# genometools/vstree

Measured on AMD Instinct MI355X. Metric: queries/sec (100 bp queries, vmatch -mum -l 20 semantics, 3 Gbp ESA index resident in HBM), higher is better.
Workload: dtype u8; 1 GPU; 3 Gbp synthetic DNA index, 10 M x 100 bp queries per GPU, -mum -l 20; index_bp=3000000000, queries_per_gpu=10000000, query_len=100, minlen=20, prefixlength=13, index_bytes_hbm=115012207262, reads_in_hbm=two bits per symbol, 32 bytes per read (vsa_pack_reads), parallelism=index replicated, queries sharded x1

## Files before the change

### vstree_amd/csrc/candidate_sort.inc

```

#define VSA_CS_CAP 4096
#define VSA_CS_ITEMS (VSA_CS_CAP / VSA_BLOCK)
#define VSA_CS_BINBITS 11
#define VSA_CS_BINS (1u << VSA_CS_BINBITS)
#define VSA_CS_BINLIMIT 256
#define VSA_CS_OVERFLOW 2u

struct CsGeometry
{
  unsigned int shift, lenbits;
  uint64_t nbuckets;
};

struct CsRegions
{
  const void *vals;
  const uint64_t *keys;
  const unsigned long long *cursors;
  uint64_t cap;
  uint64_t total;
};

struct CsFirst
{
  const uint32_t *fmlen;
  const uint64_t *fmdb;
  uint64_t nq, seqoffset;
  uint32_t packbits, valbits;
};

struct CsSources
{
  CsRegions reg[2];
  CsFirst first;
};

template <typename VAL, bool SMALL>
struct CsForm
{
  using Entry = typename std::conditional<SMALL, uint64_t, ulonglong2>::type;

  static __device__ __forceinline__ Entry make(uint64_t key, VAL val,
                                               const CsGeometry &g)
  {
    if constexpr (SMALL)
    {
      const uint64_t low = key & ((1ull << (g.shift + g.lenbits)) - 1);
      return (low << 32) | (uint64_t) val;
    } else
    {
      return make_ulonglong2(key, (uint64_t) val);
    }
  }
  static __device__ __forceinline__ uint64_t sub(const Entry &e,
                                                 const CsGeometry &g)
  {
    if constexpr (SMALL)
    {
      return e >> (32 + g.lenbits);
    } else
    {
      return (e.x >> g.lenbits) & ((1ull << g.shift) - 1);
    }
  }
  static __device__ __forceinline__ uint64_t key(const Entry &e,
                                                 uint64_t bucket,
                                                 const CsGeometry &g)
  {
    if constexpr (SMALL)
    {
      return (bucket << (g.shift + g.lenbits)) | (e >> 32);
    } else
    {
      return e.x;
    }
  }
  static __device__ __forceinline__ VAL val(const Entry &e)
  {
    if constexpr (SMALL)
    {
      return (VAL) e;
    } else
    {
      return (VAL) e.y;
    }
  }
};

struct CsTiles
{
  uint32_t group[2], ngroups[2];
};

#define VSA_CS_SCATTER_BLOCK 1024
#define VSA_CS_TILE_ITEMS 8
#define VSA_CS_TILE (VSA_CS_SCATTER_BLOCK * VSA_CS_TILE_ITEMS)
#define VSA_CS_MAXBUCKETS 12288

template <typename VAL, typename Fn>
__device__ __forceinline__ void
vsa_cs_foreach(const CsRegions &r, uint64_t wg, uint32_t group, Fn fn)
{
  const VAL *vals = static_cast<const VAL *>(r.vals);
  const uint32_t wave = threadIdx.x >> 6, lane = threadIdx.x & 63u;
  const uint64_t shard = wg * group + wave;
  if (wave >= group || shard >= VSA_CURSOR_SHARDS)
  {
    return;
  }
  uint64_t count = r.cursors[shard * VSA_CURSOR_STRIDE];
  count = count < r.cap ? count : r.cap;
  const uint64_t at = shard * r.cap;
  for (uint64_t i = lane; i < count; i += 64)
  {
    fn(r.keys[at + i], vals[at + i]);
  }
}

template <typename VAL, bool SMALL>
__global__ void __launch_bounds__(VSA_CS_SCATTER_BLOCK)
k_cs_scatter(CsSources src, CsTiles t, CsGeometry g,
             uint32_t *__restrict__ counts,
             typename CsForm<VAL, SMALL>::Entry *__restrict__ staging)
{
  extern __shared__ uint32_t cs_hist[];
  const uint32_t nb = (uint32_t) g.nbuckets;
  auto bucket = [&](uint64_t key) {
    const uint64_t b = (key >> g.lenbits) >> g.shift;
    return (uint32_t) (b < nb ? b : nb - 1);
  };
  const uint32_t lane = threadIdx.x & 63u;
  auto count = [&](uint64_t key, VAL) {
    const uint32_t b = bucket(key);
    const uint64_t active = __ballot(1);
    const uint32_t b0 = (uint32_t) __builtin_amdgcn_readfirstlane((int) b);
    if (__ballot(b == b0) == active)
    {
      if ((int) lane == __ffsll((unsigned long long) active) - 1)
      {
        atomicAdd(&cs_hist[b0], (uint32_t) __popcll(active));
      }
    } else
    {
      atomicAdd(&cs_hist[b], 1u);
    }
  };
  auto place = [&](uint64_t key, VAL val) {
    const uint32_t b = bucket(key);
    const uint64_t active = __ballot(1);
    const uint32_t b0 = (uint32_t) __builtin_amdgcn_readfirstlane((int) b);
    uint32_t rank;
    if (__ballot(b == b0) == active)
    {
      uint32_t base = 0;
      if ((int) lane == __ffsll((unsigned long long) active) - 1)
      {
        base = atomicAdd(&cs_hist[b0], (uint32_t) __popcll(active));
      }
      rank = (uint32_t) __builtin_amdgcn_readfirstlane((int) base) +
             (uint32_t) __popcll(active & ((1ull << lane) - 1));
    } else
    {
      rank = atomicAdd(&cs_hist[b], 1u);
    }
    if (rank < VSA_CS_CAP)
    {
      staging[(uint64_t) b * VSA_CS_CAP + rank] =
          CsForm<VAL, SMALL>::make(key, val, g);
    }
  };
  uint64_t wg = vsa_bid();
  int set = 0;
  while (set < 2 && wg >= t.ngroups[set])
  {
    wg -= t.ngroups[set++];
  }
  const CsFirst &f = src.first;
  uint64_t key[VSA_CS_TILE_ITEMS];
  uint32_t have = 0;
  const uint64_t q0 = wg * VSA_CS_TILE + threadIdx.x;
  if (set == 2)
  {
    uint32_t len[VSA_CS_TILE_ITEMS];
#pragma unroll
    for (int u = 0; u < VSA_CS_TILE_ITEMS; u++)
    {
      const uint64_t q = q0 + (uint64_t) u * VSA_CS_SCATTER_BLOCK;
      len[u] = q < f.nq ? f.fmlen[q] : 0;
      key[u] = q < f.nq ? f.fmdb[q] : 0;
    }
#pragma unroll
    for (int u = 0; u < VSA_CS_TILE_ITEMS; u++)
    {
      key[u] = (key[u] << f.packbits) | (((1ull << f.packbits) - 1) - len[u]);
      have |= len[u] != 0 ? 1u << u : 0u;
    }
  }
  for (uint32_t b = threadIdx.x; b < nb; b += VSA_CS_SCATTER_BLOCK)
  {
    cs_hist[b] = 0;
  }
  __syncthreads();
  if (set == 2)
  {
#pragma unroll
    for (int u = 0; u < VSA_CS_TILE_ITEMS; u++)
    {
      if ((have >> u) & 1u)
      {
        count(key[u], 0);
      }
    }
  } else
  {
    vsa_cs_foreach<VAL>(set == 0 ? src.reg[0] : src.reg[1], wg, t.group[set],
                        count);
  }
  __syncthreads();
  for (uint32_t b = threadIdx.x; b < nb; b += VSA_CS_SCATTER_BLOCK)
  {
    const uint32_t c = cs_hist[b];
    if (c != 0)
    {
      cs_hist[b] = atomicAdd(&counts[b], c);
    }
  }
  __syncthreads();
  if (set == 2)
  {
#pragma unroll
    for (int u = 0; u < VSA_CS_TILE_ITEMS; u++)
    {
      if ((have >> u) & 1u)
      {
        const uint64_t q = q0 + (uint64_t) u * VSA_CS_SCATTER_BLOCK;
        place(key[u], sizeof(VAL) == 4 ? (VAL) (q << f.valbits)
                                       : (VAL) ((q + f.seqoffset) << 16));
      }
    }
  } else
  {
    vsa_cs_foreach<VAL>(set == 0 ? src.reg[0] : src.reg[1], wg, t.group[set],
                        place);
  }
}

__global__ void __launch_bounds__(VSA_BLOCK)
k_cs_scan(const uint32_t *__restrict__ counts, uint64_t nbuckets,
          uint64_t *__restrict__ starts, unsigned int *__restrict__ flag)
{
  __shared__ uint64_t sh[VSA_BLOCK / 64 + 1];
  uint64_t run = 0;
  uint32_t largest = 0;
  for (uint64_t b = 0; b < nbuckets; b += VSA_BLOCK * VSA_FT_SCANITEMS)
  {
    const uint64_t i0 = b + (uint64_t) threadIdx.x * VSA_FT_SCANITEMS;
    uint32_t v[VSA_FT_SCANITEMS];
    uint64_t mine = 0;
#pragma unroll
    for (int k = 0; k < VSA_FT_SCANITEMS; k++)
    {
      v[k] = i0 + k < nbuckets ? counts[i0 + k] : 0;
      mine += v[k];
      largest = v[k] > largest ? v[k] : largest;
    }
    uint64_t total;
    uint64_t ex = run + vsa_block_exscan<0>(mine, sh, total);
#pragma unroll
    for (int k = 0; k < VSA_FT_SCANITEMS; k++)
    {
      if (i0 + k < nbuckets)
      {
        starts[i0 + k] = ex;
      }
      ex += v[k];
    }
    run += total;
  }
  if (largest > VSA_CS_CAP)
  {
    atomicOr(flag, VSA_CS_OVERFLOW);
  }
}

template <typename VAL, bool SMALL>
__global__ void __launch_bounds__(VSA_BLOCK)
k_cs_sort(const typename CsForm<VAL, SMALL>::Entry *__restrict__ staging,
          const uint32_t *__restrict__ counts,
          const uint64_t *__restrict__ starts,
          unsigned int *__restrict__ flag, CsGeometry g, uint64_t ncand,
          uint64_t *__restrict__ k2, VAL *__restrict__ v2)
{
  using F = CsForm<VAL, SMALL>;
  using Entry = typename F::Entry;
  __shared__ Entry buf[VSA_CS_CAP];
  __shared__ uint32_t bins[VSA_CS_BINS];
  uint64_t *sh = reinterpret_cast<uint64_t *>(buf);
  uint32_t *toobig = reinterpret_cast<uint32_t *>(buf) + 32;
  const uint64_t b = vsa_bid();
  if (b >= g.nbuckets)
  {
    return;
  }
  const uint32_t c = counts[b];
  const uint64_t start = starts[b];
  if (c == 0 || c > VSA_CS_CAP || start + c > ncand)
  {
    return;
  }
  if (threadIdx.x == 0)
  {
    *toobig = (*flag & VSA_CS_OVERFLOW) != 0 ? 1u : 0u;
  }
  const unsigned int binshift =
      g.shift > VSA_CS_BINBITS ? g.shift - VSA_CS_BINBITS : 0;
  for (uint32_t k = threadIdx.x; k < VSA_CS_BINS; k += VSA_BLOCK)
  {
    bins[k] = 0;
  }
  __syncthreads();
  if (*toobig != 0)
  {
    return;
  }
  Entry e[VSA_CS_ITEMS];
#pragma unroll
  for (int k = 0; k < VSA_CS_ITEMS; k++)
  {
    const uint32_t i = k * VSA_BLOCK + threadIdx.x;
    if (i < c)
    {
      e[k] = staging[b * VSA_CS_CAP + i];
      atomicAdd(&bins[F::sub(e[k], g) >> binshift], 1u);
    }
  }
  __syncthreads();
  {
    constexpr int PER = VSA_CS_BINS / VSA_BLOCK;
    uint32_t v[PER];
    uint64_t mine = 0;
#pragma unroll
    for (int j = 0; j < PER; j++)
    {
      v[j] = bins[threadIdx.x * PER + j];
      mine += v[j];
    }
    uint64_t total;
    uint32_t ex = (uint32_t) vsa_block_exscan<0>(mine, sh, total);
#pragma unroll
    for (int j = 0; j < PER; j++)
    {
      bins[threadIdx.x * PER + j] = ex;
      ex += v[j];
    }
  }
  __syncthreads();
  {
    constexpr int PER = VSA_CS_BINS / VSA_BLOCK;
    uint32_t big = 0;
#pragma unroll
    for (int j = 0; j < PER; j++)
    {
      const uint32_t x = threadIdx.x * PER + j;
      const uint32_t end = x + 1 < VSA_CS_BINS ? bins[x + 1] : c;
      big |= end - bins[x] > VSA_CS_BINLIMIT ? 1u : 0u;
    }
    if (big != 0)
    {
      *toobig = 1;
    }
    __syncthreads();
    if (*toobig != 0)
    {
      if (threadIdx.x == 0)
      {
        atomicOr(flag, VSA_CS_OVERFLOW);
      }
      return;
    }
    __syncthreads();
  }
#pragma unroll
  for (int k = 0; k < VSA_CS_ITEMS; k++)
  {
    const uint32_t i = k * VSA_BLOCK + threadIdx.x;
    if (i < c)
    {
      buf[atomicAdd(&bins[F::sub(e[k], g) >> binshift], 1u)] = e[k];
    }
  }
  __syncthreads();
  for (uint32_t p = threadIdx.x; p < c; p += VSA_BLOCK)
  {
    const Entry m = buf[p];
    const uint64_t sm = F::sub(m, g);
    const uint32_t x = (uint32_t) (sm >> binshift);
    const uint32_t first = x > 0 ? bins[x - 1] : 0, end = bins[x];
    uint32_t r = first;
    for (uint32_t j = first; j < end; j++)
    {
      const uint64_t sj = F::sub(buf[j], g);
      r += (sj < sm || (sj == sm && j < p)) ? 1u : 0u;
    }
    if (r < c)
    {
      k2[start + r] = F::key(m, b, g);
      v2[start + r] = F::val(m);
    }
  }
}

inline CsGeometry cs_geometry(uint64_t textlen, uint64_t ncand,
                              unsigned int lenbits, unsigned int dbbits)
{
  CsGeometry g;
  const unsigned __int128 room =
      (unsigned __int128) (VSA_CS_CAP / 2) * ((unsigned __int128) textlen + 1);
  unsigned int s = 0;
  while (s < dbbits && s < 63 && ((unsigned __int128) ncand << (s + 1)) <= room)
  {
    s++;
  }
  g.shift = s;
  g.lenbits = lenbits;
  g.nbuckets = (textlen >> s) + 1;
  return g;
}

template <typename VAL>
int candidate_bucketsort(const CsSources &src, uint64_t ncand,
                         uint64_t textlen, unsigned int lenbits,
                         unsigned int dbbits, uint64_t *k2, VAL *v2,
                         unsigned int *flag, hipStream_t stream,
                         CsGeometry *used)
{
  const CsGeometry g = cs_geometry(textlen, ncand, lenbits, dbbits);
  if (g.nbuckets > VSA_CS_MAXBUCKETS)
  {
    return -100;
  }
  const bool small = sizeof(VAL) == 4 && g.shift + lenbits <= 32;
  DevBuf counts, starts, staging;
  if (counts.alloc(g.nbuckets * 4) || starts.alloc(g.nbuckets * 8) ||
      staging.alloc(g.nbuckets * VSA_CS_CAP * (small ? 8 : 16)))
  {
    return -100;
  }
  VSA_HIP(hipMemsetAsync(counts.p, 0, g.nbuckets * 4, stream));
  CsTiles t = CsTiles();
  uint64_t nwg = 0;
  for (int s = 0; s < 2; s++)
  {
    if (src.reg[s].keys != nullptr)
    {
      const uint64_t per = src.reg[s].total / VSA_CURSOR_SHARDS + 1;
      t.group[s] = (uint32_t) std::min<uint64_t>(
          std::max<uint64_t>(VSA_CS_TILE / per, 1), VSA_CS_SCATTER_BLOCK / 64);
      t.ngroups[s] = (VSA_CURSOR_SHARDS + t.group[s] - 1) / t.group[s];
      nwg += t.ngroups[s];
    }
  }
  if (src.first.fmlen != nullptr)
  {
    nwg += (src.first.nq + VSA_CS_TILE - 1) / VSA_CS_TILE;
  }
  const dim3 sg = vsa_grid(nwg), bg = vsa_grid(g.nbuckets);
  auto run = [&](auto sm) {
    using F = CsForm<VAL, decltype(sm)::value>;
    using Entry = typename F::Entry;
    k_cs_scatter<VAL, decltype(sm)::value>
        <<<sg, VSA_CS_SCATTER_BLOCK, g.nbuckets * 4, stream>>>(
            src, t, g, counts.as<uint32_t>(), staging.as<Entry>());
    k_cs_scan<<<1, VSA_BLOCK, 0, stream>>>(counts.as<uint32_t>(), g.nbuckets,
                                           starts.as<uint64_t>(), flag);
    k_cs_sort<VAL, decltype(sm)::value><<<bg, VSA_BLOCK, 0, stream>>>(
        staging.as<Entry>(), counts.as<uint32_t>(), starts.as<uint64_t>(),
        flag, g, ncand, k2, v2);
  };
  if constexpr (sizeof(VAL) == 4)
  {
    if (small)
    {
      run(std::true_type());
    } else
    {
      run(std::false_type());
    }
  } else
  {
    run(std::false_type());
  }
  VSA_HIP(hipGetLastError());
  *used = g;
  return 0;
}
```

### vstree_amd/csrc/esa_search.hip

```cpp
#include "search_host.hpp"
#include <rocprim/rocprim.hpp>
#include <type_traits>

#include "search_complete.inc"
#include "search_query.inc"
#include "mum_workplan.inc"
#include "mem_workplan.inc"
#include "mum_filter.inc"
#include "candidate_sort.inc"
#include <atomic>


namespace
{


enum class Form
{
  Ref,
  Deep,
  Staged,
  Rows,
  Windows
};
// ... 642 lines not shown
        ix.lcp, ix.suf, index->n, st.searchlength, index->repbits);
    VSA_HIP(hipGetLastError());
    index->repleast = st.searchlength;
  }
  const Form first = pickform(index, st.queries, st.qs, Stage::MemFirst,
                              st.searchlength);
  PlanEmit em;
  if (alloc_first(st) || first_pass(st, ix, first, nullptr) ||
      plan_emit(st, VSA_PLAN_ROUNDS, &em))
  {
    return -100;
  }
  k_mem_plan<IDX><<<gridfor(nq), VSA_BLOCK, 0, st.stream>>>(
      ix, st.qs, st.perquery, st.searchlength, st.wfirste.as<uint32_t>(),
      st.wfmdb.as<uint64_t>(), index->repbits, st.wcount.as<uint32_t>(),
      st.wplan.as<PlanRanges>(), em);
  VSA_HIP(hipGetLastError());
  VSA_HIP(plan_summary(st));
  st.fromplan = true;
  st.plansearches = nq;
  return 0;
}

int dump_planfile(QueryRun &st, const char *pf)
{
  const uint64_t k = std::min<uint64_t>(st.queries->nq, 65536);
  std::vector<uint32_t> hc(k), hp(k * VSA_PLAN_RANGES);
  VSA_HIP(hipMemcpyAsync(hc.data(), st.wcount.p, k * 4,
                         hipMemcpyDeviceToHost, st.stream));
  VSA_HIP(hipMemcpyAsync(hp.data(), st.wplan.p, k * sizeof(PlanRanges),
                         hipMemcpyDeviceToHost, st.stream));
  VSA_HIP(hipStreamSynchronize(st.stream));
  if (FILE *f = fopen(pf, "wb"))
  {
    for (uint64_t q = 0; q < k; q++)
    {
      (void) fwrite(&hc[q], 4, 1, f);
      (void) fwrite(&hp[q * VSA_PLAN_RANGES], 4, VSA_PLAN_RANGES, f);
    }
    fclose(f);
  }
  return 0;
}

template <typename IDX>
int mum_plan(QueryRun &st, const DevIndex<IDX> &ix)
{
  const uint64_t nq = st.queries->nq;
  if (alloc_first(st) || st.wlist.alloc(nq * 4))
  {
    return -100;
  }
  VSA_HIP(hipMemsetAsync(st.wcount.as<uint32_t>() + nq, 0, 4, st.stream));
  const uint64_t nb = blocksfor(nq), nbr = vsa_grid_blocks(nb);
  DevBuf bcount;
  if (bcount.alloc((nbr + 1) * 8) || st.wboffset.alloc((nbr + 1) * 8))
  {
    return -100;
  }
  VSA_HIP(hipMemsetAsync(bcount.as<uint64_t>() + nb, 0, 8, st.stream));
  if (first_pass(st, ix, st.form, bcount.as<uint64_t>()))
  {
    return -100;
  }
  VSA_HIP(rocprim_run(st.wtemp, [&](void *p, size_t &tb) {
    return rocprim::exclusive_scan(p, tb, bcount.as<uint64_t>(),
                                   st.wboffset.as<uint64_t>(), (uint64_t) 0,
                                   (size_t) (nb + 1), rocprim::plus<uint64_t>(),
                                   st.stream);
  }));
  k_wanted_fill<<<vsa_grid(nb), VSA_BLOCK, 0, st.stream>>>(
      st.wcount.as<uint32_t>(), nq, 0u, st.wboffset.as<uint64_t>(),
      st.wlist.as<uint32_t>());
  VSA_HIP(hipGetLastError());
  st.nlistword = st.wboffset.as<uint64_t>() + nb;
  PlanEmit em = PlanEmit();
  if (st.form != Form::Ref && plan_emit(st, VSA_PLAN_ROUNDS - 1, &em))
  {
    return -100;
  }
  withform(st.form, [&](auto deep, auto, auto rows, auto) {
    k_mum_plan<IDX, deep, deep, rows><<<gridfor(nq), VSA_BLOCK, 0, st.stream>>>(
        ix, st.qs, st.wlist.as<uint32_t>(), st.nlistword, st.searchlength,
        st.wfirste.as<uint32_t>(), st.wcount.as<uint32_t>(),
        st.wplan.as<PlanRanges>(), em);
  });
  if (st.planemit)
  {
    VSA_HIP(plan_summary(st));
  }
  VSA_HIP(hipGetLastError());
  const char *pf = getenv("VSA_DEBUG_PLANFILE");
  if (pf != nullptr && dump_planfile(st, pf))
  {
    return -100;
  }
  st.fromplan = true;
  return 0;
}

template <typename IDX>
void launch_search(QueryRun &st, const DevIndex<IDX> &ix,
                   uint64_t nplanblocks)
{
  withform(st.form, [&](auto deep, auto, auto rows, auto) {
    auto planned = [&](auto mum) {
      k_query_search_planned<IDX, 256, deep, rows, mum>
          <<<vsa_grid(nplanblocks), 256, 0, st.stream>>>(
              ix, st.qs, st.dbase, st.perquery, st.wplan.as<PlanRanges>(),
              st.wcount.as<uint32_t>(), st.searchlength,
              st.rawout.as<vsa_match>(), st.rawkeys.as<uint64_t>(),
              st.shardcap, VSA_CURSOR_SHARDS - 1,
              st.cursor.as<unsigned long long>(), st.rec.packbits,
              st.rec.valbits, st.blocksum.as<unsigned long long>());
    };
    auto unplanned = [&](auto mum) {
      k_query_search<IDX, mum, deep, 256>
          <<<vsa_grid((st.nitems + 255) / 256), 256, 0, st.stream>>>(
              ix, st.qs, st.dbase, st.perquery, st.nitems, st.searchlength,
              st.rawout.as<vsa_match>(), st.rawkeys.as<uint64_t>(),
              st.shardcap, VSA_CURSOR_SHARDS - 1,
              st.cursor.as<unsigned long long>(), st.rec.packbits,
              st.rec.valbits);
    };
    if (st.fromplan && st.domum)
    {
      planned(std::true_type());
    } else if (st.fromplan)
    {
      if constexpr (deep && !rows)
      {
        planned(std::false_type());
      }
    } else if (st.nitems > 0 && st.domum)
    {
      unplanned(std::true_type());
    } else if (st.nitems > 0)
    {
      unplanned(std::false_type());
    }
  });
}

template <typename IDX>
int search(QueryRun &st, const DevIndex<IDX> &ix)
{
  const uint32_t nshards = VSA_CURSOR_SHARDS;
  const uint64_t nplanblocks = (st.queries->nq + 255) / 256;
  size_t rbytes = 0;
  if (st.fromplan)
  {
    if (st.blocksum.alloc((vsa_grid_blocks(nplanblocks) + 1) * 8))
    {
      return -100;
    }
    VSA_HIP(rocprim::reduce(nullptr, rbytes,
                            st.blocksum.as<unsigned long long>(),
                            (unsigned long long *) nullptr, 0ull,
                            (size_t) nplanblocks,
                            rocprim::plus<unsigned long long>(), st.stream));
    if (st.rtemp.alloc(rbytes))
    {
      return -100;
    }
  }
  if (st.cursor.alloc((size_t) nshards * VSA_CURSOR_STRIDE * 8) ||
      st.doff.alloc(nshards * 8) || st.summary.alloc(5 * 8))
  {
    return -100;
  }
  st.shardcap =
      std::max<uint64_t>((st.queries->nq * 2 / nshards) * 5 / 4 + 64, 256);
  uint64_t maxshard = 0;
  for (int attempt = 0; attempt < 2; attempt++)
  {
    if (st.rawout.alloc(nshards * st.shardcap * st.rec.recsize) ||
        st.rawkeys.alloc(nshards * st.shardcap * 8))
    {
      return -100;
    }
    VSA_HIP(hipMemsetAsync(st.cursor.p, 0,
                           (size_t) nshards * VSA_CURSOR_STRIDE * 8,
                           st.stream));
    st.tsearch.start();
    launch_search(st, ix, nplanblocks);
    st.tsearch.stop();
    VSA_HIP(hipGetLastError());
    if (st.fromplan)
    {
      VSA_HIP(rocprim::reduce(st.rtemp.p, rbytes,
                              st.blocksum.as<unsigned long long>(),
                              st.summary.as<unsigned long long>() + 4, 0ull,
                              (size_t) nplanblocks,
                              rocprim::plus<unsigned long long>(), st.stream));
    }
    const uint64_t *sm = st.summary.as<uint64_t>();
    VSA_HIP(shard_summary(st.cursor.as<unsigned long long>(), nshards,
                          st.doff.as<uint64_t>(), st.summary.as<uint64_t>(),
                          st.stream));
    const Fetch f[7] = {{sm, 8}, {sm + 1, 8}, {sm + 2, 8}, {sm + 3, 8},
                        {sm + 4, 8}, {st.planemit ? st.psummary.p : sm, 8},
                        {st.nlistword != nullptr ? st.nlistword : sm, 8}};
    uint64_t got[7];
    if (fetchwords(st.stream, f, 7, got))
    {
      return -100;
    }
    if (st.nlistword != nullptr)
    {
      st.nfirst = got[6] >> 32;
      st.plansearches = 2 * (got[6] & 0xFFFFFFFFull);
    }
    st.nplan = st.planemit ? got[5] : 0;
    st.needed = got[0];
    maxshard = got[1];
    st.plannedwork = st.fromplan ? got[4] : 0;
    st.searchms += st.tsearch.ms();
    if (maxshard <= st.shardcap)
    {
      return 0;
    }
    st.shardcap = maxshard;
  }
  VSA_ERROR("match buffer overflow: %llu > %llu",
            (unsigned long long) maxshard, (unsigned long long) st.shardcap);
  return -5;
}

int compact(QueryRun &st)
{
  const uint64_t total = st.needed + st.nplan + st.nfirst;
  if (total == 0)
  {
    return 0;
  }
  if (st.out.alloc(total * st.rec.recsize) || st.keys.alloc(total * 8) ||
      (st.nplan > 0 &&
       compact_into(st.rec, st.prawout, st.prawkeys, st.pcap, st.pcursor,
                    st.pdoff, st.out, st.keys, st.needed, st.stream)) ||
      (st.needed > 0 &&
       compact_into(st.rec, st.rawout, st.rawkeys, st.shardcap, st.cursor,
                    st.doff, st.out, st.keys, 0, st.stream)))
  {
    return -100;
  }
  if (st.nfirst > 0)
  {
    k_append_first<<<gridfor(st.queries->nq), VSA_BLOCK, 0, st.stream>>>(
        st.wfmlen.as<uint32_t>(), st.wfmdb.as<uint64_t>(),
        st.wboffset.as<uint64_t>(), st.queries->nq, st.perquery, st.dbase,
        st.qs.seqoffset, st.needed + st.nplan, st.out.as<vsa_match>(),
        st.keys.as<uint64_t>(), st.rec.packbits, st.rec.valbits);
    VSA_HIP(hipGetLastError());
  }
  st.needed = total;
  return 0;
}

#define VSA_CS_MINPAIRS (1u << 14)

std::atomic<uint64_t> g_cs_runs{0}, g_cs_overflows{0}, g_cs_longruns{0},
    g_cs_shift{0}, g_cs_buckets{0};

bool feedsbuckets(const QueryRun &st)
{
  const uint64_t total = st.needed + st.nplan + st.nfirst;
  const uint32_t tune = st.index->tune;
  if (!(st.domum && !st.domumcand && st.rec.packed && (tune & 4u) == 0 &&
        total > 0 && (total >= VSA_CS_MINPAIRS || (tune & 8u) != 0) &&
        cs_geometry(st.index->n, total, st.rec.lenbits, st.rec.dbbits)
                .nbuckets <= VSA_CS_MAXBUCKETS))
  {
    return false;
  }
  if ((tune & 8u) == 0 && st.index->cs_skip > 0)
  {
    st.index->cs_skip--;
    return false;
  }
  return true;
}

template <typename VAL>
int mumfilter_buckets(QueryRun &st, DevBuf &mums, MumCounts *c)
{
  const RecordForm &rec = st.rec;
  const uint64_t total = st.needed + st.nplan + st.nfirst;
  CsSources src = CsSources();
  if (st.needed > 0)
  {
    src.reg[0] = {st.rawout.p, st.rawkeys.as<uint64_t>(),
                  st.cursor.as<unsigned long long>(), st.shardcap, st.needed};
  }
  if (st.nplan > 0)
  {
    src.reg[1] = {st.prawout.p, st.prawkeys.as<uint64_t>(),
                  st.pcursor.as<unsigned long long>(), st.pcap, st.nplan};
  }
  if (st.nfirst > 0)
  {
    src.first = {st.wfmlen.as<uint32_t>(), st.wfmdb.as<uint64_t>(),
                 st.queries->nq, st.qs.seqoffset, rec.packbits, rec.valbits};
  }
  SortedPairs s;
  CsGeometry g;
  if (s.alloc(total, sizeof(VAL), mums))
  {
    return -100;
  }
  VSA_HIP(hipMemsetAsync(s.flag.p, 0, 8, st.stream));
  if (candidate_bucketsort<VAL>(src, total, st.index->n, rec.lenbits,
                                rec.dbbits, s.k2.as<uint64_t>(),
                                s.v2.as<VAL>(), s.flag.as<unsigned int>(),
                                st.stream, &g))
  {
    return -100;
  }
  g_cs_runs++;
  g_cs_shift = g.shift;
  g_cs_buckets = g.nbuckets;
  const PairRecord<VAL> pr = {rec.lenbits, rec.valbits,
                              sizeof(VAL) == 4 ? st.qs.seqoffset : 0};
  return mumfilter_tiles<false>(s, rec.lenbits, 0, pr, st.stream, mums, c);
}

int finish(QueryRun &st, vsa_result *res, uint64_t *mumsum)
{
  const RecordForm &rec = st.rec;
  bool allbits = false;
  if (feedsbuckets(st))
  {
    DevBuf mums;
    MumCounts c;
    if (rec.valbits != 0 ? mumfilter_buckets<uint32_t>(st, mums, &c)
                         : mumfilter_buckets<uint64_t>(st, mums, &c))
    {
      return -100;
    }
    if (c.flags == 0)
    {
      st.index->cs_penalty = 0;
      res->stats.candidates = st.needed + st.nplan + st.nfirst;
      res->count = c.nmums;
      res->matches = (vsa_match *) mums.release();
      *mumsum = c.sumlength;
      return 0;
    }
    if ((c.flags & VSA_CS_OVERFLOW) != 0)
    {
      g_cs_overflows++;
      st.index->cs_penalty =
          std::min(64u, std::max(1u, 2 * st.index->cs_penalty));
      st.index->cs_skip = st.index->cs_penalty;
    } else
    {
      g_cs_longruns++;
      allbits = true;
    }
  }
  if (compact(st))
  {
    return -100;
  }
  const uint64_t needed = st.needed;
  res->stats.candidates = st.domum ? needed : 0;
  if (rec.keeppairs)
  {
    res->count = needed;
    res->packbits = rec.lenbits;
    if (needed > 0)
    {
      res->matches = (vsa_match *) st.keys.release();
      res->packvals = (uint64_t *) st.out.release();
    }
  } else if (st.domum && !st.domumcand)
  {
    DevBuf mums;
    MumCounts c = MumCounts();
    int rc;
    if (rec.valbits != 0)
    {
      rc = mumfilter_packed(
          st.keys.as<const uint64_t>(), st.out.as<const uint32_t>(), needed,
          PairRecord<uint32_t>{rec.lenbits, rec.valbits, st.qs.seqoffset},
          rec.dbbits, 0, allbits, st.stream, mums, &c);
    } else if (rec.packed)
    {
      rc = mumfilter_packed(st.keys.as<const uint64_t>(),
                            st.out.as<const uint64_t>(), needed,
                            PairRecord<uint64_t>{rec.lenbits, 0, 0},
                            rec.dbbits, 0, allbits, st.stream, mums, &c);
    } else
    {
      rc = mumuniqueinquery(st.out, needed, st.stream, mums, &c.nmums,
                            &c.sumlength, 0, st.index->n,
                            st.queries->maxlength);
    }
    if (rc != 0)
    {
      return -100;
    }
    *mumsum = c.sumlength;
    res->count = c.nmums;
    res->matches = (vsa_match *) mums.release();
  } else if (needed > 0 && !st.ordered && st.domum)
  {
    res->count = needed;
    res->matches = (vsa_match *) st.out.release();
  } else if (needed > 0)
  {
    DevBuf sk, sm;
    if (sk.alloc(needed * 8) || sm.alloc(needed * sizeof(vsa_match)) ||
        sortbykey(st.keys.as<uint64_t>(), sk.as<uint64_t>(),
                  st.out.as<vsa_match>(), sm.as<vsa_match>(), needed,
                  bitsfor(st.nitems), st.stream))
    {
      return -100;
    }
    res->count = needed;
    res->matches = (vsa_match *) sm.release();
  }
  return 0;
}

template <typename IDX>
int run_query(const vsa_index *index, const vsa_queries *queries, bool domum,
              bool domumcand, uint32_t searchlength, vsa_result *res,
              bool ordered = true, uint32_t forcebits = 0)
{
  vsa_dev_set_stream(index->stream);
  QueryRun st(index, queries, domum, domumcand, ordered, searchlength);
  const DevIndex<IDX> ix = index->view<IDX>();
  if (workitems<IDX>(st))
  {
    return -100;
  }
  res->stats.searches = st.nitems;
  if (st.nitems == 0)
  {
    return 0;
  }
  st.tall.start();
  if (const int rc = recordform(index, queries, domum, domumcand, ordered,
                                forcebits, &st.rec))
  {
    return rc;
  }
  if (decide(st) || (st.memplan && mem_plan(st, ix)) ||
      (st.reduce && mum_plan(st, ix)))
  {
    return -100;
  }
  if (const int rc = search(st, ix))
  {
    return rc;
  }
  uint64_t mumsum = ~0ull;
  if (finish(st, res, &mumsum))
  {
    return -100;
  }
  st.tall.stop();
  VSA_HIP(hipStreamSynchronize(st.stream));
  res->stats.count = res->count;
  res->stats.search_kernel_ms = st.searchms;
  res->stats.anchor_ms = 0;
  res->stats.first_kernel_ms = st.tfirst.ms();
  res->stats.kernel_searches = st.fromplan ? st.plannedwork : st.nitems;
  if (st.fromplan)
  {
    res->stats.searches = st.plannedwork + queries->nq + st.plansearches;
  }
  res->stats.total_device_ms = st.tall.ms();
  if (mumsum != ~0ull)
  {
    res->stats.sumlength = mumsum;
    return 0;
  }
  if (st.rec.keeppairs)
  {
    res->stats.sumlength = 0;
    return 0;
  }
  return sumlengths(res->matches, res->count, st.stream,
                    &res->stats.sumlength);
}

template <typename Limits, typename Run>
int query_entry(const char *name, const vsa_index *index,
                const vsa_queries *queries, const uint64_t *searchlength,
                vsa_result **result, Limits limits, Run run)
{
  if (index == nullptr || queries == nullptr || result == nullptr)
  {
    VSA_ERROR("%s: NULL argument", name);
    return -1;
  }
  *result = nullptr;
  if (queries->device != index->device)
  {
    VSA_ERROR("queries live on device %d, index on device %d",
              queries->device, index->device);
    return -1;
  }
  if (index->bck == nullptr)
  {
    VSA_ERROR("table bck is not loaded");
    return -3;
  }
  if (searchlength != nullptr && *searchlength < index->pl)
  {
    VSA_ERROR("searchlength=%lu must be >= %lu=prefixlen",
              (unsigned long) *searchlength, (unsigned long) index->pl);
    return -2;
  }
  if (const int rc = limits())
  {
    return rc;
  }
  if (vsa_set_device(index->device) != 0)
  {
    return -100;
  }
  vsa_result *res = newresult(index->device);
  const int rc =
      (index->isize == 4) ? run(uint32_t(), res) : run(uint64_t(), res);
  if (rc != 0)
  {
    vsa_result_free(res);
    return rc;
  }
  *result = res;
  return 0;
}

int mumlimit(const vsa_index *index, uint64_t searchlength)
{
  if (searchlength > 0xFFFFFFF0ull)
  {
    VSA_ERROR("searchlength=%lu must be >= %lu=prefixlen",
              (unsigned long) searchlength, (unsigned long) index->pl);
    return -2;
  }
  return 0;
}

}


extern "C" int vsa_findcompletematches(const vsa_index *index,
                                       const vsa_queries *queries,
                                       vsa_result **result)
{
  uint64_t qlimit = 0;
  bool shortquery = false;
  const int rc = query_entry(
      "vsa_findcompletematches", index, queries, nullptr, result,
      [&] {
        if (queries->maxlength > 0xFFFFFFF0ull)
        {
          VSA_ERROR("query length beyond 32 bits is not supported");
          return -3;
        }
        return 0;
      },
      [&](auto idx, vsa_result *res) {
        qlimit = queries->nq;
        if (queries->minlength < index->pl)
        {
          for (uint64_t q = 0; q < queries->nq; q++)
          {
            if (queries->hlength[q] < index->pl)
            {
              qlimit = q;
              shortquery = true;
              break;
            }
          }
        }
        return run_complete<decltype(idx)>(index, queries, qlimit, res);
      });
  if (rc == 0 && shortquery)
  {
    VSA_ERROR("patternlength=%lu must be >= %lu=prefixlen",
              (unsigned long) queries->hlength[qlimit],
              (unsigned long) index->pl);
    return -2;
  }
  return rc;
}

extern "C" int vsa_findmumcandidates(const vsa_index *index,
                                     const vsa_queries *queries,
                                     uint64_t searchlength, int ordered,
                                     vsa_result **result)
{
  if (ordered)
  {
    return vsa_findquerymatches(index, queries, 1, 1, searchlength, result);
  }
  return query_entry(
      "vsa_findmumcandidates", index, queries, &searchlength, result,
      [&] { return mumlimit(index, searchlength); },
      [&](auto idx, vsa_result *res) {
        return run_query<decltype(idx)>(index, queries, true, true,
                                        (uint32_t) searchlength, res, false);
      });
}

extern "C" int vsa_findmumcandidates_packed(const vsa_index *index,
                                            const vsa_queries *queries,
                                            uint64_t searchlength,
                                            uint32_t lengthbits,
                                            vsa_result **result)
{
  return query_entry(
      "vsa_findmumcandidates_packed", index, queries, &searchlength, result,
      [&] {
        if (const int rc = mumlimit(index, searchlength))
        {
          return rc;
        }
        if (lengthbits == 0)
        {
          lengthbits = bitsfor(queries->maxlength);
        }
// ... 226 lines not shown
```

Before: 3.325 billion queries/s.

## Fuse MUM containment filter into per-bucket candidate sort, drop global sorted pairs

The bucket sort no longer writes a fully sorted key/value array for a separate mumfilter_tiles pass. Each bucket block now sorts its candidates in shared memory, applies the containment filter directly, and compacts the survivors back into staging. A cross-bucket carry (an atomicMax of right ends, recorded during scatter) handles intervals that span buckets. A scan over survivor counts then drives a write kernel that emits matches directly. This removes the global k2/v2 round trip and the separate filter kernels, at the cost of a per-candidate atomicMax loop over the spanned buckets and a host fetch of the totals.

```diff
diff --git a/vstree_amd/csrc/candidate_sort.inc b/vstree_amd/csrc/candidate_sort.inc
--- a/vstree_amd/csrc/candidate_sort.inc
+++ b/vstree_amd/csrc/candidate_sort.inc
@@ -121,9 +121,11 @@
 __global__ void __launch_bounds__(VSA_CS_SCATTER_BLOCK)
 k_cs_scatter(CsSources src, CsTiles t, CsGeometry g,
              uint32_t *__restrict__ counts,
+             unsigned long long *__restrict__ bcarry,
              typename CsForm<VAL, SMALL>::Entry *__restrict__ staging)
 {
   extern __shared__ uint32_t cs_hist[];
+  const KeyToRightEnd rightend = {g.lenbits};
   const uint32_t nb = (uint32_t) g.nbuckets;
   auto bucket = [&](uint64_t key) {
     const uint64_t b = (key >> g.lenbits) >> g.shift;
@@ -168,6 +170,13 @@
       staging[(uint64_t) b * VSA_CS_CAP + rank] =
           CsForm<VAL, SMALL>::make(key, val, g);
     }
+    const uint64_t end = rightend(key);
+    uint64_t last = end >> g.shift;
+    last = last < nb ? last : nb - 1;
+    for (uint64_t later = (uint64_t) b + 1; later <= last; later++)
+    {
+      atomicMax(&bcarry[later], (unsigned long long) end);
+    }
   };
   uint64_t wg = vsa_bid();
   int set = 0;
@@ -245,56 +254,34 @@
   }
 }
 
-__global__ void __launch_bounds__(VSA_BLOCK)
-k_cs_scan(const uint32_t *__restrict__ counts, uint64_t nbuckets,
-          uint64_t *__restrict__ starts, unsigned int *__restrict__ flag)
-{
-  __shared__ uint64_t sh[VSA_BLOCK / 64 + 1];
-  uint64_t run = 0;
-  uint32_t largest = 0;
-  for (uint64_t b = 0; b < nbuckets; b += VSA_BLOCK * VSA_FT_SCANITEMS)
-  {
-    const uint64_t i0 = b + (uint64_t) threadIdx.x * VSA_FT_SCANITEMS;
-    uint32_t v[VSA_FT_SCANITEMS];
-    uint64_t mine = 0;
-#pragma unroll
-    for (int k = 0; k < VSA_FT_SCANITEMS; k++)
-    {
-      v[k] = i0 + k < nbuckets ? counts[i0 + k] : 0;
-      mine += v[k];
-      largest = v[k] > largest ? v[k] : largest;
-    }
-    uint64_t total;
-    uint64_t ex = run + vsa_block_exscan<0>(mine, sh, total);
-#pragma unroll
-    for (int k = 0; k < VSA_FT_SCANITEMS; k++)
-    {
-      if (i0 + k < nbuckets)
-      {
-        starts[i0 + k] = ex;
-      }
-      ex += v[k];
-    }
-    run += total;
-  }
-  if (largest > VSA_CS_CAP)
-  {
-    atomicOr(flag, VSA_CS_OVERFLOW);
-  }
+__device__ __forceinline__ uint64_t vsa_wave_inclusive_max(uint64_t v)
+{
+  const uint32_t lane = threadIdx.x & 63u;
+#pragma unroll
+  for (int d = 1; d < 64; d <<= 1)
+  {
+    const uint64_t o =
+        vsa_shfl64(v, (int) (lane >= (uint32_t) d ? lane - d : lane));
+    v = lane >= (uint32_t) d && o > v ? o : v;
+  }
+  return v;
 }
 
 template <typename VAL, bool SMALL>
 __global__ void __launch_bounds__(VSA_BLOCK)
-k_cs_sort(const typename CsForm<VAL, SMALL>::Entry *__restrict__ staging,
-          const uint32_t *__restrict__ counts,
-          const uint64_t *__restrict__ starts,
-          unsigned int *__restrict__ flag, CsGeometry g, uint64_t ncand,
-          uint64_t *__restrict__ k2, VAL *__restrict__ v2)
+k_cs_filter(typename CsForm<VAL, SMALL>::Entry *__restrict__ staging,
+            const uint32_t *__restrict__ counts,
+            const unsigned long long *__restrict__ bcarry,
+            unsigned int *__restrict__ flag, CsGeometry g, uint64_t carry,
+            uint64_t *__restrict__ bsurv, uint64_t *__restrict__ blen)
 {
   using F = CsForm<VAL, SMALL>;
   using Entry = typename F::Entry;
+  constexpr uint32_t SEGS = VSA_CS_ITEMS * (VSA_BLOCK / 64);
+  static_assert(SEGS <= 64, "the first wavefront scans the segments");
   __shared__ Entry buf[VSA_CS_CAP];
-  __shared__ uint32_t bins[VSA_CS_BINS];
+  __shared__ uint64_t binwords[VSA_CS_BINS / 2];
+  uint32_t *bins = reinterpret_cast<uint32_t *>(binwords);
   uint64_t *sh = reinterpret_cast<uint64_t *>(buf);
   uint32_t *toobig = reinterpret_cast<uint32_t *>(buf) + 32;
   const uint64_t b = vsa_bid();
@@ -303,9 +290,16 @@
     return;
   }
   const uint32_t c = counts[b];
-  const uint64_t start = starts[b];
-  if (c == 0 || c > VSA_CS_CAP || start + c > ncand)
-  {
+  if (c == 0)
+  {
+    return;
+  }
+  if (c > VSA_CS_CAP)
+  {
+    if (threadIdx.x == 0)
+    {
+      atomicOr(flag, VSA_CS_OVERFLOW);
+    }
     return;
   }
   if (threadIdx.x == 0)
@@ -323,40 +317,43 @@
   {
     return;
   }
-  Entry e[VSA_CS_ITEMS];
-#pragma unroll
-  for (int k = 0; k < VSA_CS_ITEMS; k++)
-  {
-    const uint32_t i = k * VSA_BLOCK + threadIdx.x;
-    if (i < c)
-    {
-      e[k] = staging[b * VSA_CS_CAP + i];
-      atomicAdd(&bins[F::sub(e[k], g) >> binshift], 1u);
-    }
-  }
-  __syncthreads();
-  {
+  auto binof = [&](const Entry &x) {
+    const uint64_t bin = F::sub(x, g) >> binshift;
+    return (uint32_t) (bin < VSA_CS_BINS ? bin : VSA_CS_BINS - 1);
+  };
+  {
+    Entry e[VSA_CS_ITEMS];
+#pragma unroll
+    for (int k = 0; k < VSA_CS_ITEMS; k++)
+    {
+      const uint32_t i = k * VSA_BLOCK + threadIdx.x;
+      if (i < c)
+      {
+        e[k] = staging[b * VSA_CS_CAP + i];
+        atomicAdd(&bins[binof(e[k])], 1u);
+      }
+    }
+    __syncthreads();
     constexpr int PER = VSA_CS_BINS / VSA_BLOCK;
-    uint32_t v[PER];
-    uint64_t mine = 0;
-#pragma unroll
-    for (int j = 0; j < PER; j++)
-    {
-      v[j] = bins[threadIdx.x * PER + j];
-      mine += v[j];
-    }
-    uint64_t total;
-    uint32_t ex = (uint32_t) vsa_block_exscan<0>(mine, sh, total);
-#pragma unroll
-    for (int j = 0; j < PER; j++)
-    {
-      bins[threadIdx.x * PER + j] = ex;
-      ex += v[j];
-    }
-  }
-  __syncthreads();
-  {
-    constexpr int PER = VSA_CS_BINS / VSA_BLOCK;
+    {
+      uint32_t v[PER];
+      uint64_t mine = 0;
+#pragma unroll
+      for (int j = 0; j < PER; j++)
+      {
+        v[j] = bins[threadIdx.x * PER + j];
+        mine += v[j];
+      }
+      uint64_t total;
+      uint32_t ex = (uint32_t) vsa_block_exscan<0>(mine, sh, total);
+#pragma unroll
+      for (int j = 0; j < PER; j++)
+      {
+        bins[threadIdx.x * PER + j] = ex;
+        ex += v[j];
+      }
+    }
+    __syncthreads();
     uint32_t big = 0;
 #pragma unroll
     for (int j = 0; j < PER; j++)
@@ -379,33 +376,217 @@
       return;
     }
     __syncthreads();
-  }
-#pragma unroll
-  for (int k = 0; k < VSA_CS_ITEMS; k++)
-  {
-    const uint32_t i = k * VSA_BLOCK + threadIdx.x;
-    if (i < c)
-    {
-      buf[atomicAdd(&bins[F::sub(e[k], g) >> binshift], 1u)] = e[k];
-    }
-  }
-  __syncthreads();
-  for (uint32_t p = threadIdx.x; p < c; p += VSA_BLOCK)
-  {
-    const Entry m = buf[p];
-    const uint64_t sm = F::sub(m, g);
-    const uint32_t x = (uint32_t) (sm >> binshift);
-    const uint32_t first = x > 0 ? bins[x - 1] : 0, end = bins[x];
-    uint32_t r = first;
-    for (uint32_t j = first; j < end; j++)
-    {
-      const uint64_t sj = F::sub(buf[j], g);
-      r += (sj < sm || (sj == sm && j < p)) ? 1u : 0u;
-    }
-    if (r < c)
-    {
-      k2[start + r] = F::key(m, b, g);
-      v2[start + r] = F::val(m);
+#pragma unroll
+    for (int k = 0; k < VSA_CS_ITEMS; k++)
+    {
+      const uint32_t i = k * VSA_BLOCK + threadIdx.x;
+      if (i < c)
+      {
+        const uint32_t at = atomicAdd(&bins[binof(e[k])], 1u);
+        if (at < c)
+        {
+          buf[at] = e[k];
+        }
+      }
+    }
+  }
+  __syncthreads();
+  {
+    Entry m[VSA_CS_ITEMS];
+    uint32_t place[VSA_CS_ITEMS];
+#pragma unroll
+    for (int k = 0; k < VSA_CS_ITEMS; k++)
+    {
+      const uint32_t p = k * VSA_BLOCK + threadIdx.x;
+      place[k] = VSA_CS_CAP;
+      if (p < c)
+      {
+        m[k] = buf[p];
+        const uint64_t sm = F::sub(m[k], g);
+        const uint32_t x = binof(m[k]);
+        uint32_t first = x > 0 ? bins[x - 1] : 0, end = bins[x];
+        end = end < c ? end : c;
+        uint32_t r = first;
+        for (uint32_t j = first; j < end; j++)
+        {
+          const uint64_t sj = F::sub(buf[j], g);
+          r += (sj < sm || (sj == sm && j < p)) ? 1u : 0u;
+        }
+        place[k] = r;
+      }
+    }
+    __syncthreads();
+#pragma unroll
+    for (int k = 0; k < VSA_CS_ITEMS; k++)
+    {
+      if (place[k] < c)
+      {
+        buf[place[k]] = m[k];
+      }
+    }
+  }
+  __syncthreads();
+  uint64_t *segmax = binwords;
+  uint32_t *segcount = bins + 128;
+  uint64_t *sh2 = binwords + 128;
+  const KeyToRightEnd rightend = {g.lenbits};
+  const uint64_t lenmask = (1ull << g.lenbits) - 1;
+  const uint32_t lane = threadIdx.x & 63u, wave = threadIdx.x >> 6;
+  const uint32_t nsegs = (c + VSA_BLOCK - 1) / VSA_BLOCK * (VSA_BLOCK / 64);
+  auto keyat = [&](uint32_t i) { return F::key(buf[i], b, g); };
+  uint64_t before[VSA_CS_ITEMS];
+#pragma unroll
+  for (int r = 0; r < VSA_CS_ITEMS; r++)
+  {
+    before[r] = 0;
+    if ((uint32_t) r * VSA_BLOCK < c)
+    {
+      const uint32_t i = r * VSA_BLOCK + threadIdx.x;
+      const uint64_t incl =
+          vsa_wave_inclusive_max(i < c ? rightend(keyat(i)) : 0);
+      const uint64_t prev = vsa_shfl64(incl, (int) (lane > 0 ? lane - 1 : 0));
+      before[r] = lane > 0 ? prev : 0;
+      if (lane == 63)
+      {
+        segmax[r * (VSA_BLOCK / 64) + wave] = incl;
+      }
+    }
+  }
+  __syncthreads();
+  if (threadIdx.x < 64)
+  {
+    const uint64_t incl =
+        vsa_wave_inclusive_max(lane < nsegs ? segmax[lane] : 0);
+    const uint64_t prev = vsa_shfl64(incl, (int) (lane > 0 ? lane - 1 : 0));
+    uint64_t start = bcarry[b];
+    start = carry > start ? carry : start;
+    const uint64_t mine = lane > 0 ? prev : 0;
+    segmax[lane] = mine > start ? mine : start;
+  }
+  __syncthreads();
+  uint32_t okbits = 0;
+  uint64_t len = 0;
+#pragma unroll
+  for (int r = 0; r < VSA_CS_ITEMS; r++)
+  {
+    if ((uint32_t) r * VSA_BLOCK < c)
+    {
+      const uint32_t i = r * VSA_BLOCK + threadIdx.x;
+      bool ok = false;
+      uint64_t kk = 0;
+      if (i < c)
+      {
+        kk = keyat(i);
+        const uint64_t e = rightend(kk);
+        const uint64_t seg = segmax[r * (VSA_BLOCK / 64) + wave];
+        const uint64_t run = seg > before[r] ? seg : before[r];
+        ok = run < e;
+        if (ok)
+        {
+          const uint64_t d = kk >> g.lenbits;
+          uint32_t steps = 0;
+          for (uint32_t j = i; j > 0 && (keyat(j - 1) >> g.lenbits) == d; j--)
+          {
+            if (rightend(keyat(j - 1)) >= e || ++steps > VSA_RUN_LIMIT)
+            {
+              ok = false;
+              break;
+            }
+          }
+          if (steps > VSA_RUN_LIMIT)
+          {
+            atomicOr(flag, 1u);
+          }
+          steps = 0;
+          for (uint32_t j = i + 1;
+               ok && j < c && (keyat(j) >> g.lenbits) == d; j++)
+          {
+            if (rightend(keyat(j)) >= e || ++steps > VSA_RUN_LIMIT)
+            {
+              ok = false;
+            }
+          }
+          if (steps > VSA_RUN_LIMIT)
+          {
+            atomicOr(flag, 1u);
+          }
+        }
+      }
+      const uint64_t mask = __ballot(ok);
+      if (lane == 0)
+      {
+        segcount[r * (VSA_BLOCK / 64) + wave] = (uint32_t) __popcll(mask);
+      }
+      okbits |= ok ? 1u << r : 0u;
+      len += ok ? lenmask - (kk & lenmask) : 0;
+    }
+  }
+  __syncthreads();
+  if (threadIdx.x < 64)
+  {
+    const uint32_t v = lane < nsegs ? segcount[lane] : 0;
+    uint32_t incl = v;
+#pragma unroll
+    for (int d = 1; d < 64; d <<= 1)
+    {
+      const uint32_t o = __shfl_up(incl, d, 64);
+      incl += lane >= (uint32_t) d ? o : 0;
+    }
+    segcount[lane] = incl - v;
+    if (lane == 63)
+    {
+      segcount[SEGS] = incl;
+    }
+  }
+  __syncthreads();
+#pragma unroll
+  for (int r = 0; r < VSA_CS_ITEMS; r++)
+  {
+    if ((uint32_t) r * VSA_BLOCK < c)
+    {
+      const bool ok = ((okbits >> r) & 1u) != 0;
+      const uint64_t mask = __ballot(ok);
+      const uint32_t at = segcount[r * (VSA_BLOCK / 64) + wave] +
+                          (uint32_t) __popcll(mask & ((1ull << lane) - 1));
+      if (ok && at < c)
+      {
+        staging[b * VSA_CS_CAP + at] = buf[r * VSA_BLOCK + threadIdx.x];
+      }
+    }
+  }
+  uint64_t alllen;
+  (void) vsa_block_exscan<0>(len, sh2, alllen);
+  if (threadIdx.x == 0)
+  {
+    const uint32_t kept = segcount[SEGS];
+    bsurv[b] = kept < c ? kept : c;
+    blen[b] = alllen;
+  }
+}
+
+template <typename VAL, bool SMALL>
+__global__ void __launch_bounds__(VSA_BLOCK)
+k_cs_write(const typename CsForm<VAL, SMALL>::Entry *__restrict__ staging,
+           const uint64_t *__restrict__ bsurv, const uint64_t *__restrict__ off,
+           CsGeometry g, uint64_t ncand, PairRecord<VAL> write,
+           vsa_match *__restrict__ out)
+{
+  using F = CsForm<VAL, SMALL>;
+  const uint64_t b = vsa_bid();
+  if (b >= g.nbuckets)
+  {
+    return;
+  }
+  uint64_t n = bsurv[b];
+  n = n < VSA_CS_CAP ? n : VSA_CS_CAP;
+  const uint64_t at = off[b];
+#pragma unroll 4
+  for (uint64_t i = threadIdx.x; i < n; i += VSA_BLOCK)
+  {
+    if (at + i < ncand)
+    {
+      const typename F::Entry e = staging[b * VSA_CS_CAP + i];
+      write(F::key(e, b, g), (uint64_t) F::val(e), out + at + i);
     }
   }
 }
@@ -428,11 +609,11 @@
 }
 
 template <typename VAL>
-int candidate_bucketsort(const CsSources &src, uint64_t ncand,
-                         uint64_t textlen, unsigned int lenbits,
-                         unsigned int dbbits, uint64_t *k2, VAL *v2,
-                         unsigned int *flag, hipStream_t stream,
-                         CsGeometry *used)
+int candidate_bucketfilter(const CsSources &src, uint64_t ncand,
+                           uint64_t textlen, unsigned int lenbits,
+                           unsigned int dbbits, uint64_t carry,
+                           PairRecord<VAL> write, hipStream_t stream,
+                           vsa_match *out, uint64_t got[3], CsGeometry *used)
 {
   const CsGeometry g = cs_geometry(textlen, ncand, lenbits, dbbits);
   if (g.nbuckets > VSA_CS_MAXBUCKETS)
@@ -440,13 +621,21 @@
     return -100;
   }
   const bool small = sizeof(VAL) == 4 && g.shift + lenbits <= 32;
-  DevBuf counts, starts, staging;
-  if (counts.alloc(g.nbuckets * 4) || starts.alloc(g.nbuckets * 8) ||
-      staging.alloc(g.nbuckets * VSA_CS_CAP * (small ? 8 : 16)))
+  const uint64_t nb = g.nbuckets;
+  const uint64_t zeroed = (2 + 3 * nb + (nb + 1) / 2 + 1) & ~1ull;
+  DevBuf words, staging;
+  if (words.alloc((zeroed + 2 * (nb + 1)) * 8) ||
+      staging.alloc(nb * VSA_CS_CAP * (small ? 8 : 16)))
   {
     return -100;
   }
-  VSA_HIP(hipMemsetAsync(counts.p, 0, g.nbuckets * 4, stream));
+  uint64_t *w = words.as<uint64_t>();
+  unsigned int *flag = reinterpret_cast<unsigned int *>(w);
+  unsigned long long *bcarry = reinterpret_cast<unsigned long long *>(w + 2);
+  uint64_t *bsurv = w + 2 + nb, *blen = w + 2 + 2 * nb;
+  uint32_t *counts = reinterpret_cast<uint32_t *>(w + 2 + 3 * nb);
+  uint64_t *off = w + zeroed, *lenscan = off + nb + 1;
+  VSA_HIP(hipMemsetAsync(w, 0, zeroed * 8, stream));
   CsTiles t = CsTiles();
   uint64_t nwg = 0;
   for (int s = 0; s < 2; s++)
@@ -464,18 +653,19 @@
   {
     nwg += (src.first.nq + VSA_CS_TILE - 1) / VSA_CS_TILE;
   }
-  const dim3 sg = vsa_grid(nwg), bg = vsa_grid(g.nbuckets);
+  const dim3 sg = vsa_grid(nwg), bg = vsa_grid(nb);
   auto run = [&](auto sm) {
     using F = CsForm<VAL, decltype(sm)::value>;
     using Entry = typename F::Entry;
     k_cs_scatter<VAL, decltype(sm)::value>
-        <<<sg, VSA_CS_SCATTER_BLOCK, g.nbuckets * 4, stream>>>(
-            src, t, g, counts.as<uint32_t>(), staging.as<Entry>());
-    k_cs_scan<<<1, VSA_BLOCK, 0, stream>>>(counts.as<uint32_t>(), g.nbuckets,
-                                           starts.as<uint64_t>(), flag);
-    k_cs_sort<VAL, decltype(sm)::value><<<bg, VSA_BLOCK, 0, stream>>>(
-        staging.as<Entry>(), counts.as<uint32_t>(), starts.as<uint64_t>(),
-        flag, g, ncand, k2, v2);
+        <<<sg, VSA_CS_SCATTER_BLOCK, nb * 4, stream>>>(
+            src, t, g, counts, bcarry, staging.as<Entry>());
+    k_cs_filter<VAL, decltype(sm)::value><<<bg, VSA_BLOCK, 0, stream>>>(
+        staging.as<Entry>(), counts, bcarry, flag, g, carry, bsurv, blen);
+    k_mumf_scan<0><<<2, VSA_BLOCK, 0, stream>>>(bsurv, nb, 0, off, blen,
+                                                lenscan);
+    k_cs_write<VAL, decltype(sm)::value><<<bg, VSA_BLOCK, 0, stream>>>(
+        staging.as<Entry>(), bsurv, off, g, ncand, write, out);
   };
   if constexpr (sizeof(VAL) == 4)
   {
@@ -491,6 +681,11 @@
     run(std::false_type());
   }
   VSA_HIP(hipGetLastError());
+  const Fetch f[3] = {{off + nb, 8}, {lenscan + nb, 8}, {flag, 8}};
+  if (fetchwords(stream, f, 3, got))
+  {
+    return -100;
+  }
   *used = g;
   return 0;
 }
diff --git a/vstree_amd/csrc/esa_search.hip b/vstree_amd/csrc/esa_search.hip
--- a/vstree_amd/csrc/esa_search.hip
+++ b/vstree_amd/csrc/esa_search.hip
@@ -968,26 +968,27 @@
     src.first = {st.wfmlen.as<uint32_t>(), st.wfmdb.as<uint64_t>(),
                  st.queries->nq, st.qs.seqoffset, rec.packbits, rec.valbits};
   }
-  SortedPairs s;
   CsGeometry g;
-  if (s.alloc(total, sizeof(VAL), mums))
-  {
-    return -100;
-  }
-  VSA_HIP(hipMemsetAsync(s.flag.p, 0, 8, st.stream));
-  if (candidate_bucketsort<VAL>(src, total, st.index->n, rec.lenbits,
-                                rec.dbbits, s.k2.as<uint64_t>(),
-                                s.v2.as<VAL>(), s.flag.as<unsigned int>(),
-                                st.stream, &g))
+  if (mums.alloc(total * sizeof(vsa_match)))
+  {
+    return -100;
+  }
+  const PairRecord<VAL> pr = {rec.lenbits, rec.valbits,
+                              sizeof(VAL) == 4 ? st.qs.seqoffset : 0};
+  uint64_t got[3];
+  if (candidate_bucketfilter<VAL>(src, total, st.index->n, rec.lenbits,
+                                  rec.dbbits, 0, pr, st.stream,
+                                  mums.as<vsa_match>(), got, &g))
   {
     return -100;
   }
   g_cs_runs++;
   g_cs_shift = g.shift;
   g_cs_buckets = g.nbuckets;
-  const PairRecord<VAL> pr = {rec.lenbits, rec.valbits,
-                              sizeof(VAL) == 4 ? st.qs.seqoffset : 0};
-  return mumfilter_tiles<false>(s, rec.lenbits, 0, pr, st.stream, mums, c);
+  c->nmums = got[0];
+  c->sumlength = got[1];
+  c->flags = got[2];
+  return 0;
 }
 
 int finish(QueryRun &st, vsa_result *res, uint64_t *mumsum)
```

Result: faster. 3.382 billion queries/s (median of 6 runs) (+1.7%).
